# kowallus/mbgc

Hardware: AMD Instinct MI355X
Metric: input Gbases/s (compress hot path, -m1: match-finding + stream emission) (higher is better)
Workload: dtype u8

## Files before the change

### mbgc_amd/binding.py

```python
import ctypes as C
import os

import numpy as np

HERE = os.path.dirname(os.path.abspath(__file__))
LIB_PATH = os.environ.get("MBGC_HIP_LIB", os.path.join(HERE, "libmbgc_hip.so"))
NO_LOCK = 2 ** 64 - 1
SKIPPED = 2 ** 64 - 1
STREAM_NAMES = ("literals", "mapOff", "mapOff5th", "mapLen", "gapDelta", "flags")
KERNEL_FAMILIES = ("load", "insert", "probe", "emit2", "resolve", "stitch", "emit")

EXPORTS = """swsem_last_error swsem_device_count swsem_device_numa_node swsem_create swsem_destroy swsem_set_stream swsem_synchronize
swsem_disable_sliding_window swsem_set_sliding_window_size swsem_disable_circular_buffer swsem_get_ref_length
swsem_get_loading_position swsem_get_loaded_ref_length swsem_get_max_ref_length swsem_get_sliding_window_size swsem_get_dropped_bytes swsem_set_position
swsem_acquire_lock swsem_release_lock swsem_get_K swsem_get_hash_size swsem_load_ref swsem_load_ref_dev
swsem_load_separator swsem_finalize_targets swsem_revcomp_dev swsem_match swsem_match_batch_dev swsem_batch_counts swsem_batch_matches
swsem_batch_fingerprint swsem_emit_params_default swsem_emit swsem_emit_batch swsem_emit_batch_begin swsem_emit_batch_begin_spec swsem_emit_batch_end swsem_emit_select swsem_emit_result swsem_emit_set_host_copy swsem_emit_unmatched swsem_emit_pack_dev swsem_emit_pack_dev_on swsem_emit_counters swsem_debug_copy_ref swsem_debug_write_ref swsem_debug_copy_ht swsem_debug_emit_stats
swsem_profile_enable swsem_profile_get swsem_batch_stats swsem_dev_malloc swsem_dev_free swsem_dev_upload swsem_dev_download swsem_dev_copy swsem_decode_contigs_dev swsem_emit_verify
swsem_create_decoder swsem_decode_plan_chain_dev swsem_decode_fill_range_dev swsem_decode_load_dev""".split()


class SpecFinalize(C.Structure):
    _fields_ = [("ntargets", C.c_int), ("ext_dev", C.c_void_p), ("ext_len", C.POINTER(C.c_uint64)), ("addSep", C.c_int), ("sep", C.c_int),
                ("lazySeparator", C.c_int), ("lockPos", C.POINTER(C.c_uint64)), ("loadedAfter", C.POINTER(C.c_uint64)),
# ... 122 lines not shown
        L.swsem_profile_get.argtypes = [vp, C.POINTER(C.c_double), pu64]
        L.swsem_batch_stats.argtypes = [vp, pu64]
        _lib = L
    return _lib


def _chk(rc):
    if rc != 0:
        raise SwsemError("swsem error %d: %s" % (rc, lib().swsem_last_error().decode()))


def _bytes_ptr(a):
    a = np.ascontiguousarray(a, dtype=np.uint8)
    return a, a.ctypes.data_as(C.c_void_p)


def emit_params(mode=1, **over):
    p = EmitParams()
    lib().swsem_emit_params_default(C.byref(p), mode)
    for k, v in over.items():
        setattr(p, k, v)
    return p


class SlidingWindowSparseEMMatcher:

    def __init__(self, max_ref_len, L=32, k1=16, k2=1, skip_margin=16, device=0):
        self.h = C.c_void_p()
        _chk(lib().swsem_create(C.byref(self.h), max_ref_len, L, k1, k2, skip_margin, device))

    def close(self):
        if getattr(self, "h", None):
            lib().swsem_destroy(self.h)
            self.h = None

    def __del__(self):
        self.close()

    def disable_sliding_window(self): lib().swsem_disable_sliding_window(self.h)
    def set_sliding_window_size(self, f): lib().swsem_set_sliding_window_size(self.h, f)
    def disable_circular_buffer(self): lib().swsem_disable_circular_buffer(self.h)
    def ref_length(self): return lib().swsem_get_ref_length(self.h)
    def loading_position(self): return lib().swsem_get_loading_position(self.h)
    def loaded_ref_length(self): return lib().swsem_get_loaded_ref_length(self.h)
    def max_ref_length(self): return lib().swsem_get_max_ref_length(self.h)
    def sliding_window_size(self): return lib().swsem_get_sliding_window_size(self.h)
    def dropped_bytes(self): return lib().swsem_get_dropped_bytes(self.h)

    def emit_stats(self):
        out = (C.c_uint64 * 8)()
        lib().swsem_debug_emit_stats.argtypes = [C.c_void_p, C.POINTER(C.c_uint64)]
        _chk(lib().swsem_debug_emit_stats(self.h, out))
        return {"foreign_boundary_steps": int(out[4]), "blocks_not_accepted": int(out[5]), "groups_replayed": int(out[6]),
                "blocks_given_up": int(out[7])}
    def set_position(self, pos, laps): lib().swsem_set_position(self.h, pos, laps)
    def acquire_lock(self): return lib().swsem_acquire_lock(self.h)
    def release_lock(self, v): _chk(lib().swsem_release_lock(self.h, v)); return 0
    def hash_size(self): return lib().swsem_get_hash_size(self.h)
    def K(self): return lib().swsem_get_K(self.h)
    def set_stream(self, stream_ptr): _chk(lib().swsem_set_stream(self.h, stream_ptr))
    def synchronize(self): _chk(lib().swsem_synchronize(self.h))

    def load_ref(self, text, load_rc=False, add_sep=True, sep=0):
        a, p = _bytes_ptr(text)
        _chk(lib().swsem_load_ref(self.h, p, a.size, int(load_rc), int(add_sep), sep))

    def load_ref_dev(self, dev_ptr, n, load_rc=False, add_sep=True, sep=0):
        _chk(lib().swsem_load_ref_dev(self.h, dev_ptr, n, int(load_rc), int(add_sep), sep))

    def load_separator(self, sep=0): _chk(lib().swsem_load_separator(self.h, sep))

    def finalize_targets(self, ext_ptrs, ext_lens, locks, lazy=True, add_sep=True, sep=0):
        n = len(ext_lens)
        ptrs = (C.c_void_p * n)(*[int(p) for p in ext_ptrs])
        lens = np.ascontiguousarray(ext_lens, dtype=np.uint64)
        lk = np.ascontiguousarray(locks, dtype=np.uint64)
        out = np.zeros(n, dtype=np.uint64)
        P = C.POINTER(C.c_uint64)
        _chk(lib().swsem_finalize_targets(self.h, n, ptrs, lens.ctypes.data_as(P), int(add_sep), sep, int(lazy),
                                          lk.ctypes.data_as(P), out.ctypes.data_as(P)))
        return out
    def revcomp_dev(self, src_ptr, n, dst_ptr): _chk(lib().swsem_revcomp_dev(self.h, src_ptr, n, dst_ptr))

    def match(self, q, min_len=32, lock=NO_LOCK):
        a, p = _bytes_ptr(q)
        out, n = C.c_void_p(), C.c_uint64()
        _chk(lib().swsem_match(self.h, p, a.size, min_len, lock, C.byref(out), C.byref(n)))
        if n.value == 0:
            return np.zeros((0, 3), dtype=np.uint64)
        return np.ctypeslib.as_array(C.cast(out, C.POINTER(C.c_uint64)), shape=(n.value, 3)).copy()

    def match_batch_dev(self, dev_ptr, offsets, min_len=32, locks=None):
        offs = np.ascontiguousarray(offsets, dtype=np.uint64)
        n = offs.size - 1
        lk = None
        if locks is not None:
            lk = np.ascontiguousarray(locks, dtype=np.uint64)
            assert lk.size == n
        _chk(lib().swsem_match_batch_dev(self.h, dev_ptr, offs.ctypes.data_as(C.POINTER(C.c_uint64)), n, min_len,
                                         lk.ctypes.data_as(C.POINTER(C.c_uint64)) if lk is not None else None))
        self._batch_n = n

    def batch_counts(self):
        out = np.zeros(self._batch_n, dtype=np.uint64)
        _chk(lib().swsem_batch_counts(self.h, out.ctypes.data_as(C.POINTER(C.c_uint64))))
        return out

# ... 190 lines not shown
```

### mbgc_amd/csrc/swsem_emit.hip

```cpp
#include "swsem_device.h"
#include "../../include/mbgc_swsem.h"

namespace swk {

constexpr int EMIT_THREADS = 1024;
constexpr uint8_t MATCH_MARK = 0xA5;
constexpr int MAX_EXTEND_MATCH_LEFT_LENGTH = 1 << 24;

struct EMatch {
    uint64_t posSrc, len, posDest, lp;
};

struct EmitContig {
    uint64_t qoff, n;
    uint64_t matchBase;
    uint64_t lock;
    uint64_t scratchBase;
    uint64_t streamBase[SWSEM_NSTREAMS];
    uint32_t cap;
    uint32_t chunk0;
    int32_t factor;
    uint32_t span0;
    int64_t processed, targetIdx;
};

struct EmitOut {
    uint64_t size[SWSEM_NSTREAMS];
    uint64_t unmatchedChars;
    uint64_t extMatched, extMismatches, totalMatched, removed, nmatches;
};

struct LongCopy { uint8_t *dst; const uint8_t *src; uint64_t len; };
constexpr uint32_t LONG_COPY_CAP = 4096;
constexpr uint32_t LONG_COPY_MIN = 32768;

struct EmitView {
    const uint8_t *ref, *qbuf;
    const Match *matches;
    const uint32_t *matchCount;
    uint64_t pos1, refLength, maxRefLength;
    const uint64_t *loaded; uint32_t nLoaded;
    swsem_emit_params_t p;
    EMatch *em;
    uint64_t *next0;
    uint8_t *removed;
    uint32_t *keepIdx;
    uint32_t *meta;
    uint32_t *corr;
    unsigned long long *pairMask;
    unsigned long long *litBits;
    unsigned long long *metaBad;
    uint32_t *sz;
    uint32_t *ofs;
    uint32_t *chunkCnt;
    const uint32_t *chunkOwner;
    const uint32_t *spanOwner;
    uint32_t ncontigs;
    uint64_t *packBase;
    uint8_t *arena;
    struct LongCopy *longCopies;
    uint32_t *longCount;
    EmitOut *out;
};

constexpr uint32_t META_SKIPOFF = 1, META_HASGAP = 2, META_ISGAP = 4, META_GSTART = 8, META_GMID = 16, META_GEND = 32;

__device__ __forceinline__ bool paired(uint64_t aSrc, uint64_t aDst, uint64_t bSrc, uint64_t bDst) {
    return aSrc + bDst == bSrc + aDst;
}

__device__ __forceinline__ int sym5(uint8_t c) {
    return c == 'A' ? 0 : c == 'C' ? 1 : c == 'G' ? 2 : c == 'T' ? 3 : c == 'N' ? 4 : -1;
}
__device__ __forceinline__ uint8_t mismatch2code(uint8_t actual, uint8_t mismatch) {
    const int a = sym5(actual), b = sym5(mismatch);
    if (actual == mismatch || a < 0 || b < 0) return mismatch;
    const uint32_t rows[5] = {0 | 2u << 3 | 0u << 6 | 1u << 9 | 3u << 12, 1 | 0u << 3 | 2u << 6 | 0u << 9 | 3u << 12,
                              0 | 2u << 3 | 0u << 6 | 1u << 9 | 3u << 12, 1 | 0u << 3 | 2u << 6 | 0u << 9 | 3u << 12,
                              1 | 2u << 3 | 3u << 6 | 0u << 9 | 0u << 12};
    return (uint8_t) ((rows[a] >> (3 * b)) & 7u);
}

__device__ __forceinline__ uint64_t loaded_pos(const EmitView &v, uint64_t pos) {
    const uint64_t span = v.refLength - 1;
    const uint64_t back = v.loaded[v.nLoaded - 1];
    while (pos + span < back) pos += span;
    return pos;
}

template <int NT>
__device__ uint32_t block_scan(uint32_t x, uint32_t *lds, uint32_t *total) {
    const uint32_t lane = threadIdx.x & (WAVE - 1), w = threadIdx.x / WAVE;
    uint32_t inc = x;
    for (int d = 1; d < WAVE; d <<= 1) {
        const uint32_t y = (uint32_t) __shfl_up((int) inc, d);
        if ((int) lane >= d) inc += y;
    }
    __syncthreads();
    if (lane == WAVE - 1) lds[w] = inc;
    __syncthreads();
    if (threadIdx.x == 0) {
        uint32_t run = 0;
        for (int i = 0; i < NT / WAVE; i++) { const uint32_t t = lds[i]; lds[i] = run; run += t; }
// ... 285 lines not shown
                                    (gs ? META_GSTART : 0) | (gm ? META_GMID : 0) | (ge ? META_GEND : 0) | (gapByte << 8);
                metaV = wl32(mw, k, metaV);
                corrV = wl32(isGap ? (uint32_t) st.gapStartIdx : (uint32_t) j, k, corrV);
            }
        }
        if (WRITE && lane < cnt) {
            v.meta[cg.scratchBase + jl] = metaV;
            v.corr[cg.scratchBase + jl] = corrV;
        }
        st.nxA = st.nxB;
        st.nxB = 0;
    }
}


__device__ __forceinline__ bool mrec_equal(const MetaRec &a, const MetaRec &b) {
    uint32_t ra, rb;
    __builtin_memcpy(&ra, a.rel, 4); __builtin_memcpy(&rb, b.rel, 4);
    uint64_t d = (a.claimed ^ b.claimed) | (uint64_t) (a.gapStartIdx ^ b.gapStartIdx) | (uint64_t) (a.gapEndIdx ^ b.gapEndIdx) |
                 (uint64_t) (a.flags ^ b.flags) | (uint64_t) (ra ^ rb);
#pragma unroll
    for (int e = 0; e < MNX; e++) d |= a.val[e] ^ b.val[e];
    return d == 0;
}

__device__ __forceinline__ void mrec_store(MetaRec *dst, unsigned long long claimed, bool cur, int gs, int ge, const int (&nxPos)[MNX],
                                           const uint64_t (&nxVal)[MNX], bool overflow, int J) {
    uint32_t r[MNX]; uint64_t x[MNX];
#pragma unroll
    for (int e = 0; e < MNX; e++) { r[e] = nxPos[e] >= J ? (uint32_t) (nxPos[e] - J) : 0xFFu; x[e] = nxPos[e] >= J ? nxVal[e] : 0; }
    auto cx = [&](int a, int b) {
        if (r[a] > r[b]) { const uint32_t t = r[a]; r[a] = r[b]; r[b] = t; const uint64_t u = x[a]; x[a] = x[b]; x[b] = u; }
    };
    cx(0, 1); cx(2, 3); cx(0, 2); cx(1, 3); cx(1, 2);
    MetaRec R;
    R.claimed = claimed; R.gapStartIdx = gs; R.gapEndIdx = ge;
    R.flags = (cur ? MREC_CUR : 0u) | (overflow ? MREC_OVERFLOW : 0u);
#pragma unroll
    for (int e = 0; e < MNX; e++) { R.rel[e] = (uint8_t) r[e]; R.val[e] = x[e]; }
    *dst = R;
}

struct MetaSpan { uint32_t gk; int n, B0; bool live; };
__device__ __forceinline__ MetaSpan meta_span(const EmitView &v, const EmitContig *__restrict__ cgs) {
    MetaSpan sp;
    sp.gk = v.spanOwner[blockIdx.x];
    const EmitOut o = v.out[sp.gk];
    sp.n = (int) o.nmatches;
    sp.B0 = (int) (blockIdx.x - cgs[sp.gk].span0) * MSPAN;
    sp.live = o.unmatchedChars != UINT64_MAX && sp.B0 < sp.n;
    return sp;
}

__global__ void __launch_bounds__(CH) k_emit_meta_regions(EmitView v, const EmitContig *__restrict__ cgs) {
    if (!v.p.lazyDecompressionSupport) return;
    const uint32_t gk = v.chunkOwner[blockIdx.x];
    const EmitContig cg = cgs[gk];
    const uint32_t gx = blockIdx.x - cg.chunk0;
    const EmitOut o = v.out[gk];
    if (o.unmatchedChars == UINT64_MAX) return;
    const uint64_t t = (uint64_t) gx * CH + threadIdx.x;
    if (t >= o.nmatches) return;
    const uint64_t lp = loaded_pos(v, v.em[cg.scratchBase + t].posSrc);
    v.em[cg.scratchBase + t].lp = lp;
    uint32_t lo = 0, hi = v.nLoaded;
    while (lo < hi) { const uint32_t mid = (lo + hi) / 2; if (v.loaded[mid] <= lp) lo = mid + 1; else hi = mid; }
    v.next0[cg.scratchBase + t] = lo == v.nLoaded ? UINT64_MAX : v.loaded[lo];
}

__global__ void __launch_bounds__(MLANES) k_emit_meta_masks(EmitView v, const EmitContig *__restrict__ cgs) {
    __shared__ uint64_t skey[MPAD_SIZE], slp[MPAD_SIZE];
    const MetaSpan sp = meta_span(v, cgs);
    if (!sp.live) return;
    const EmitContig cg = cgs[sp.gk];
    const int n = sp.n, B0 = sp.B0, tid = (int) threadIdx.x;
    const int P1 = B0 + MSPAN < n ? B0 + MSPAN : n;
    const int PK = P1 + WAVE < n ? P1 + WAVE : n;
    const EMatch *E = v.em + cg.scratchBase;
    const bool lazy = v.p.lazyDecompressionSupport != 0;
    const int depth = v.p.gapDepthOffsetEncoding;
    for (int i = tid; i < ((PK - B0 + WAVE - 1) & ~(WAVE - 1)); i += MLANES) {
        const int m = B0 + i;
        bool lit0 = false;
        if (m < PK) {
            const EMatch e = E[m];
            const uint64_t side = e.posSrc > cg.lock ? 1u : (e.posSrc < cg.lock ? 2u : 0u);
            skey[mpad(i)] = ((e.posSrc - e.posDest) << 2) | side;
            slp[mpad(i)] = e.lp;
            const uint64_t nxt = m + 1 < n ? E[m + 1].posDest : cg.n;
            lit0 = nxt - (uint32_t) (e.posDest + e.len) == 0;
        }
        const unsigned long long lb = __ballot(lit0);
        if ((tid & (WAVE - 1)) == 0 && m < P1) v.litBits[(size_t) cg.chunk0 * (CH / WAVE) + (size_t) (m / WAVE)] = lb;
    }
    __syncthreads();
    for (int i = tid; i < P1 - B0; i += MLANES) {
        const int m = B0 + i;
        const int gCnt = n - m - 1 < depth ? n - m - 1 : depth;
        const uint64_t kj = skey[mpad(i)];
        const uint64_t own = lazy ? v.next0[cg.scratchBase + m] : UINT64_MAX;
        unsigned long long pm = 0;
#pragma unroll 8
        for (int g = 1; g <= WAVE; g++) {
            const int x = mpad(g <= gCnt ? i + g : i);
            const bool ok = (g <= gCnt) & (skey[x] == kj) & ((slp[x] < own) | !lazy);
            pm |= (unsigned long long) ok << (g - 1);
        }
        v.pairMask[cg.scratchBase + m] = pm;
    }
}

__global__ void __launch_bounds__(MLANES) k_emit_meta_spec(EmitView v, const EmitContig *__restrict__ cgs, MetaRec *__restrict__ recs, int warm,
                                                          unsigned long long *__restrict__ stats) {
    __shared__ uint64_t spm[MPAD_SIZE], sown[MPAD_SIZE];
    __shared__ unsigned long long slit[MPAD_N / WAVE + 2];
    const MetaSpan sp = meta_span(v, cgs);
    if (!sp.live) return;
    const EmitContig cg = cgs[sp.gk];
    const int n = sp.n, B0 = sp.B0, tid = (int) threadIdx.x;
    const int P0 = B0 >= MWARM ? B0 - MWARM : 0;
    const int P1 = B0 + MSPAN < n ? B0 + MSPAN : n;
    const EMatch *E = v.em + cg.scratchBase;
    const bool lazy = v.p.lazyDecompressionSupport != 0, ext = v.p.enableExtensionsWithMismatches != 0;
    const int depth = v.p.gapDepthOffsetEncoding, depthMism = v.p.gapDepthMismatchesEncoding;
    const int PK = P1 + WAVE < n ? P1 + WAVE : n;
    for (int i = tid; i < PK - P0; i += MLANES) {
        if (P0 + i < P1) spm[mpad(i)] = v.pairMask[cg.scratchBase + P0 + i];
        sown[mpad(i)] = lazy ? v.next0[cg.scratchBase + P0 + i] : 0;
    }
    if (tid < MPAD_N / WAVE + 2) {
        const int w = P0 / WAVE + tid;
        slit[tid] = w * WAVE < P1 ? v.litBits[(size_t) cg.chunk0 * (CH / WAVE) + (size_t) w] : 0;
    }
    __syncthreads();
    const int j0 = B0 + tid * MB;
    const bool active = j0 < n;
    const int j1 = j0 + MB < n ? j0 + MB : n;
    unsigned long long claimed = 0;
    bool cur = false, overflow = false;
    int gs = -1, ge = -1;
    int nxPos[MNX]; uint64_t nxVal[MNX];
#pragma unroll
    for (int e = 0; e < MNX; e++) { nxPos[e] = -1; nxVal[e] = 0; }
    MetaRec *myRecs = recs + ((size_t) cg.chunk0 * (CH / MB) + (size_t) (j0 / MB)) * 2;
    for (int s = 0; s < MWARM + MB; s++) {
        const int j = j0 - MWARM + s;
        if (s == MWARM && active) mrec_store(myRecs, claimed, cur, gs, ge, nxPos, nxVal, overflow, j0);
        if (!active || j < j0 - warm || j < 0 || j >= j1) continue;
        const int i = j - P0;
        if (ext && j == ge) { gs = -1; ge = -1; }
        const bool skipOffset = cur;
        const int gCnt = n - j - 1 < depth ? n - j - 1 : depth;
        const bool rule = !lazy && gs == -1 && ((slit[i / WAVE] >> (i & (WAVE - 1))) & 1);
        const unsigned long long taken = claimed | (rule ? 1ull : 0ull);
        unsigned long long em = spm[mpad(i)] & ~taken;
        uint64_t inherited = 0;
#pragma unroll
        for (int e = 0; e < MNX; e++) if (nxPos[e] == j) { inherited = nxVal[e]; nxPos[e] = -1; }
        uint64_t nextj = 0;
        if (lazy) {
            nextj = sown[mpad(i)];
            if (inherited && inherited != nextj) {
                nextj = inherited;
                atomicAdd(&stats[4], 1ull);
                const EMatch mj = E[j];
                em = 0;
                for (int g = 1; g <= gCnt; g++) {
                    const EMatch c = E[j + g];
                    const bool pw = paired(mj.posSrc, mj.posDest, c.posSrc, c.posDest) &&
                                    ((mj.posSrc > cg.lock && c.posSrc > cg.lock) || (mj.posSrc < cg.lock && c.posSrc < cg.lock));
                    if (pw && c.lp < nextj) em |= 1ull << (g - 1);
                }
                em &= ~taken;
            }
        }
        uint32_t gapByte = 0;
        if (em) {
            const int gf = __builtin_ctzll(em) + 1;
            const unsigned long long below = gf > 1 ? ((1ull << (gf - 1)) - 1) : 0ull;
            gapByte = (uint32_t) (gf - __popcll(taken & below));
            claimed |= 1ull << (gf - 1);
            if (lazy && nextj != sown[mpad(i + gf)]) {
                bool put = false;
#pragma unroll
                for (int e = 0; e < MNX; e++) if (!put && nxPos[e] < 0) { nxPos[e] = j + gf; nxVal[e] = nextj; put = true; }
                overflow |= !put;
            }
            if (ext && ge <= j + gf && gf <= depthMism) { gs = j; ge = j + gf; }
        }
        cur = claimed & 1ull;
        claimed >>= 1;
        if (j >= j0) {
            const bool s0 = gs == j, e0 = ge == j + 1, m0 = gs < j && j + 1 < ge;
            const bool isGap = s0 || m0 || e0;
            const uint32_t mw = (skipOffset ? META_SKIPOFF : 0) | (gCnt ? META_HASGAP : 0) | (isGap ? META_ISGAP : 0) |
                                (s0 ? META_GSTART : 0) | (m0 ? META_GMID : 0) | (e0 ? META_GEND : 0) | (gapByte << 8);
            v.meta[cg.scratchBase + j] = mw;
            v.corr[cg.scratchBase + j] = (uint32_t) (isGap ? gs : j);
        }
    }
    if (active) mrec_store(myRecs + 1, claimed, cur, gs, ge, nxPos, nxVal, overflow, j1);
    if (active && overflow) atomicAdd(&stats[7], 1ull);
}

__global__ void __launch_bounds__(WAVE) k_emit_meta_check(EmitView v, const EmitContig *__restrict__ cgs, const MetaRec *__restrict__ recs,
                                                          unsigned long long *__restrict__ stats) {
    constexpr int CPW = WAVE * MB / CH;
    const uint32_t gk = v.chunkOwner[blockIdx.x];
    const EmitContig cg = cgs[gk];
    const uint32_t gx = blockIdx.x - cg.chunk0;
    if (gx % CPW) return;
    const EmitOut o = v.out[gk];
    if (o.unmatchedChars == UINT64_MAX) return;
    const int64_t n = (int64_t) o.nmatches, nblk = (n + MB - 1) / MB;
    const int64_t b = (int64_t) (gx / CPW) * WAVE + threadIdx.x;
    if (b - (int64_t) threadIdx.x >= nblk) return;
    const MetaRec *R0 = recs + (size_t) cg.chunk0 * (CH / MB) * 2;
    bool bad = false;
    if (b < nblk) {
        const MetaRec S = R0[2 * b], F = R0[2 * b + 1];
        bad = ((S.flags | F.flags) & MREC_OVERFLOW) != 0;
        if (b > 0 && !bad) bad = !mrec_equal(S, R0[2 * b - 1]);
    }
    const unsigned long long mb = __ballot(bad);
    if (threadIdx.x == 0) {
        v.metaBad[cg.chunk0 + gx / CPW] = mb;
        if (mb) atomicAdd(&stats[5], (unsigned long long) __popcll(mb));
    }
}

__device__ __forceinline__ void mrec_expand(const MetaRec &R, MetaRun &st) {
    st.claimed = rfl64(R.claimed); st.curClaimed = (rfl32(R.flags) & MREC_CUR) != 0;
    st.gapStartIdx = (int64_t) rfl64((uint64_t) R.gapStartIdx); st.gapEndIdx = (int64_t) rfl64((uint64_t) R.gapEndIdx);
    st.nxA = 0; st.nxB = 0;
#pragma unroll
// ... 743 lines not shown
```

### mbgc_amd/csrc/swsem_runtime.hip

```cpp
#include "../../include/mbgc_swsem.h"
#include "swsem_kernels.hip"
#include "swsem_resolve4.hip"
#include "swsem_emit.hip"
#include "swsem_decode.hip"

#include <algorithm>
#include <cctype>
#include <chrono>
#include <mutex>
#include <cstdarg>
#include <cstdio>
#include <cstdlib>
#include <cstring>
#include <deque>
#include <string>
#include <vector>

using namespace swk;

#include "swsem_runtime_state.h"
#include "swsem_runtime_streams.h"
#include "swsem_runtime_loader.h"
#include "swsem_runtime_match.h"
#include "swsem_runtime_emit.h"
// ... 290 lines not shown
    HIPCHK(hipGetLastError());
    return SWSEM_OK;
}

int swsem_debug_copy_ref(swsem_t *h, uint64_t from, uint64_t n, uint8_t *out) {
    HIPCHK(hipStreamSynchronize(h->stream));
    HIPCHK(hipMemcpy(out, h->ref + from, n, hipMemcpyDeviceToHost));
    return SWSEM_OK;
}

int swsem_debug_write_ref(swsem_t *h, uint64_t from, uint64_t n, const uint8_t *in) { MATCHER_ONLY(h);
    if (from + n > h->maxRefLength) return fail(SWSEM_EINVAL, "swsem_debug_write_ref: beyond the buffer");
    HIPCHK(hipStreamSynchronize(h->stream));
    HIPCHK(hipStreamSynchronize(h->stream2));
    HIPCHK(hipMemcpy(h->ref + from, in, n, hipMemcpyHostToDevice));
    {
        const uint64_t s0 = from >= (uint64_t) h->K ? (from - h->K + 1) >> h->k1ord : 0, s1 = (from + n + ((1ull << h->k1ord) - 1)) >> h->k1ord;
        if (h->tags && s1 > s0) HIPCHK(hipMemset(h->tags + s0, 0, (s1 - s0) * sizeof(uint16_t)));
    }
    return SWSEM_OK;
}

int swsem_debug_copy_ht(swsem_t *h, uint32_t *out) { MATCHER_ONLY(h);
    DevBuf<uint32_t> tmp;
    int r = tmp.reserve(h->hash_size);
    if (r) return r;
    k_ht_low_words<<<dim3((h->hash_size + 255) / 256), dim3(256), 0, h->stream>>>(h->ht, tmp.p, h->hash_size, h->fpBits);
    HIPCHK(hipStreamSynchronize(h->stream));
    HIPCHK(hipMemcpy(out, tmp.p, (size_t) h->hash_size * 4, hipMemcpyDeviceToHost));
    return SWSEM_OK;
}

int swsem_debug_block_times(swsem_t *h, uint64_t *out, uint64_t cap, uint64_t *n) { MATCHER_ONLY(h);
    uint64_t nb = 0;
    for (auto &c : h->contigs) nb += c.nrb;
    *n = nb;
    if (nb > cap) nb = cap;
    std::vector<BlockRec> tmp(nb);
    HIPCHK(hipStreamSynchronize(h->stream));
    if (nb) HIPCHK(hipMemcpy(tmp.data(), h->dRecs.p, nb * sizeof(BlockRec), hipMemcpyDeviceToHost));
    for (uint64_t i = 0; i < nb; i++) { out[3 * i] = tmp[i].cycles; out[3 * i + 1] = tmp[i].visits; out[3 * i + 2] = tmp[i].emits; }
    return SWSEM_OK;
}

int swsem_debug_emit_stats(swsem_t *h, uint64_t out[8]) { MATCHER_ONLY(h);
    HIPCHK(hipDeviceSynchronize());
    for (int k = 0; k < 8; k++) out[k] = 0;
    for (auto &E : h->slot) {
        if (!E.dEStat.p || !E.statZeroed) continue;
        unsigned long long t[8];
        HIPCHK(hipMemcpy(t, E.dEStat.p, sizeof t, hipMemcpyDeviceToHost));
        for (int k = 0; k < 8; k++) out[k] += t[k];
    }
    return SWSEM_OK;
}

#ifdef SWSEM_DIAG_PHASES
int swsem_debug_phases(swsem_t *h, uint64_t *out) {
    HIPCHK(hipStreamSynchronize(h->stream));
    unsigned long long z[8] = {0};
    HIPCHK(hipMemcpyFromSymbol(out, HIP_SYMBOL(swk::g_diag), sizeof z));
    HIPCHK(hipMemcpyToSymbol(HIP_SYMBOL(swk::g_diag), z, sizeof z));
    return SWSEM_OK;
}
#endif

int swsem_profile_enable(swsem_t *h, int on) {
    h->drain_events();
    h->prof = on != 0;
    memset(h->profMs, 0, sizeof h->profMs);
    memset(h->profN, 0, sizeof h->profN);
    return SWSEM_OK;
}

int swsem_profile_get(swsem_t *h, double ms[SWSEM_K_COUNT], uint64_t n[SWSEM_K_COUNT]) {
    h->drain_events();
    for (int i = 0; i < SWSEM_K_COUNT; i++) { ms[i] = h->profMs[i]; n[i] = h->profN[i]; }
    return SWSEM_OK;
}

int swsem_batch_stats(swsem_t *h, uint64_t s[9]) { MATCHER_ONLY(h);
    if (!h->batchValid) return fail(SWSEM_EINVAL, "no batch results");
    for (int i = 0; i < 9; i++) s[i] = h->stats[i];
    return SWSEM_OK;
}

void swsem_emit_params_default(swsem_emit_params_t *p, int mode) {
    memset(p, 0, sizeof(*p));
    p->enableExtensionsWithMismatches = 1;
    p->mismatchesWithExclusion = 1;
    p->lazyDecompressionSupport = 1;
    p->enable40bitReference = 0;
    p->frugal64bitLenEncoding = 1;
    p->gapDepthOffsetEncoding = 64;
    p->gapDepthMismatchesEncoding = 2;
    p->gapBreakingMatchMinLength = 256;
    p->mmsMatchBonus = 50;
    p->mmsMismatchPenalty = 50;
    p->mmsMismatchesScoreThreshold = 500;
    p->mmsMismatchesInitialScore = 125;
    p->allowedTargetsOutrunForDissimilarContigs = 1;
    p->minimalLengthForDissimilarContigs = 1024;
    p->unmatchedFractionFactorTweakForDissimilarContigs = 16;
    if (mode == 0) {
        p->allowedTargetsOutrunForDissimilarContigs = 4;
        p->unmatchedFractionFactorTweakForDissimilarContigs = 32;
// ... 231 lines not shown
```

### mbgc_amd/csrc/swsem_runtime_emit.h

```cpp
namespace {

int end_slot(swsem *h, int si) {
    EmitSlot &E = h->slot[si];
    if (!E.outstanding) return SWSEM_OK;
    HIPCHK(hipSetDevice(h->device));
    { int d = run_phase2b(h, E, false); if (d) return d; }
    HIPCHK(hipEventSynchronize(E.evDone));
    E.outstanding = false;
    const int n = E.emitN;
    E.eout.assign((const EmitOut *) E.pinE.p, (const EmitOut *) E.pinE.p + n);
    uint64_t tot = 0;
    E.hostStreamOff.assign((size_t) n * SWSEM_NSTREAMS, 0);
    for (int k = 0; k < n; k++)
        for (int st = 0; st < SWSEM_NSTREAMS; st++) {
            if (E.eout[k].unmatchedChars == UINT64_MAX) E.eout[k].size[st] = 0;
            E.hostStreamOff[(size_t) k * SWSEM_NSTREAMS + st] = tot;
            tot += E.eout[k].size[st];
        }
    E.packedBytes = tot;
    E.hostStreamsValid = false;
    if (h->emitHostCopy) {
        int r = E.next_host_streams(tot + 1);
        if (r) return r;
        if (tot) HIPCHK(hipMemcpyAsync(E.hostStreams().p, E.dEArena.p, tot, hipMemcpyDeviceToHost, h->s3()));
        HIPCHK(hipStreamSynchronize(h->s3()));
        E.hostStreamsValid = true;
    }
    return SWSEM_OK;
}


int emit_layout(swsem *h, EmitSlot &E, int n, const int *contigIdx, const uint64_t *lockPos, const int *factor,
                const int64_t *processed, const int64_t *targetIdx, uint64_t &rows, uint64_t &arena) {
    E.ecg.assign(n, EmitContig());
    std::vector<int> &which = E.ewhich;
    which.assign(n, 0);
    rows = 0; arena = 0;
    E.chunkOwner.clear(); E.spanOwner.clear();
    for (int k = 0; k < n; k++) {
        const int c = contigIdx ? contigIdx[k] : k;
        if (c < 0 || c >= (int) h->contigs.size()) return fail(SWSEM_EINVAL, "swsem_emit: no contig %d in the batch", c);
        which[k] = c;
        EmitContig &e = E.ecg[k];
        const Contig &cg = h->contigs[c];
        const uint64_t nm = cg.n / (h->minLen ? h->minLen : 1) + 2;
        e.qoff = cg.qoff; e.n = cg.n; e.matchBase = cg.matchBase;
        e.lock = lockPos ? lockPos[k] : UINT64_MAX;
        e.scratchBase = rows;
        e.cap = (uint32_t) (nm + 2);
        rows += e.cap;
        e.chunk0 = (uint32_t) E.chunkOwner.size();
        E.chunkOwner.insert(E.chunkOwner.end(), (e.cap + CH - 1) / CH, (uint32_t) k);
        e.span0 = (uint32_t) E.spanOwner.size();
        E.spanOwner.insert(E.spanOwner.end(), (e.cap + MSPAN - 1) / MSPAN, (uint32_t) k);
        e.factor = factor ? factor[k] : 128;
        e.processed = processed ? processed[k] : 0;
        e.targetIdx = targetIdx ? targetIdx[k] : 0;
        const uint64_t szs[SWSEM_NSTREAMS] = {cg.n + nm + 16, 4 * nm + 16, nm + 16, 14 * nm + 16, nm + 16, cg.n + 2 * nm + 16};
        for (int st = 0; st < SWSEM_NSTREAMS; st++) { e.streamBase[st] = arena; arena += (szs[st] + 15) & ~15ull; }
    }
    return SWSEM_OK;
}

int emit_reserve(swsem *h, EmitSlot &E, int n, uint64_t rows, uint64_t arena, uint64_t nLoaded) {
    h->capN = std::max<uint64_t>(h->capN, (uint64_t) n); h->capRows = std::max(h->capRows, rows); h->capArena = std::max(h->capArena, arena);
    if (nLoaded + 1 > h->capLoaded) h->capLoaded = std::max<uint64_t>(4096, 2 * (nLoaded + 1));
    h->capChunks = std::max<uint64_t>(h->capChunks, E.chunkOwner.size());
    const uint64_t N = h->capN, R = h->capRows, A = h->capArena, Cn = h->capChunks;
    int r;
    if ((r = E.dECg.reserve(N)) || (r = E.dEOut.reserve(N)) || (r = E.dEWhich.reserve(N)) || (r = E.dEM.reserve(R)) ||
        (r = E.dENext0.reserve(R)) || (r = E.dERm.reserve(R)) ||
        (r = E.dEKeep.reserve(R)) || (r = E.dEMeta.reserve(R)) || (r = E.dECorr.reserve(R)) ||
        (r = E.dESz.reserve(R * 6)) || (r = E.dEOfs.reserve(R * 6)) || (r = E.dEArena.reserve(A)) || (r = E.dELoaded.reserve(h->capLoaded)) ||
        (r = E.dEStat.reserve(8)) || (r = E.dELong.reserve(LONG_COPY_CAP)) || (r = E.dELongCount.reserve(4)) || (r = E.dEPm.reserve(R)) ||
        (r = E.dELit.reserve((size_t) Cn * (CH / WAVE))) || (r = E.dEBad.reserve(Cn)) || (r = E.dEOwner.reserve(Cn)) || (r = E.dESpanOwner.reserve(Cn)) ||
        (r = E.dEStates.reserve((size_t) Cn * (CH / MB) * 2)) || (r = E.dEChunk.reserve((size_t) Cn * 6)) ||
        (r = E.dEPack.reserve((size_t) N * SWSEM_NSTREAMS)))
        return r;
    if (!E.statZeroed) { HIPCHK(hipMemsetAsync(E.dEStat.p, 0, 8 * sizeof(unsigned long long), h->stream)); E.statZeroed = true; }
    return SWSEM_OK;
}

int emit_upload_tables(swsem *h, EmitSlot &E, int n, const uint64_t *refExtLoadedPos, uint64_t nLoaded, const swsem_spec_finalize_t *spec) {
    hipStream_t up = h->streamUp;
    int r;
    if (!h->roundTopFresh) HIPCHK(hipEventRecord(h->evRoundTop, h->stream));
    h->roundTopFresh = false;
    HIPCHK(hipStreamWaitEvent(up, h->evRoundTop, 0));
    if ((r = upload(h, E.dEOwner.p, E.chunkOwner.data(), E.chunkOwner.size() * sizeof(uint32_t), up))) return r;
    if ((r = upload(h, E.dESpanOwner.p, E.spanOwner.data(), E.spanOwner.size() * sizeof(uint32_t), up))) return r;
    if ((r = upload(h, E.dECg.p, E.ecg.data(), n * sizeof(EmitContig), up)) || (r = upload(h, E.dEWhich.p, E.ewhich.data(), n * sizeof(int), up))) return r;
    E.eloaded.assign(refExtLoadedPos, refExtLoadedPos + nLoaded);
    if ((r = upload(h, E.dELoaded.p, E.eloaded.data(), nLoaded * sizeof(uint64_t), up))) return r;
    if (spec) {
        if ((r = h->dGate.reserve(4)) || (r = h->dPred.reserve(2 * (size_t) n + 64))) return r;
        if ((r = upload(h, h->dPred.p, spec->predExt, n, up)) || (r = upload(h, h->dPred.p + n, spec->predRC, n, up))) return r;
    }
    return flush_copies(h);
}

EmitView emit_book(swsem *h, EmitSlot &E, int si, const swsem_emit_params_t *p, int n, uint64_t nLoaded) {
    EmitView v;
    v.ref = h->ref; v.qbuf = h->qdev; v.matches = h->dMatches.p; v.matchCount = h->dMatchCount.p;
    v.pos1 = (uint64_t) h->ld.pos1; v.refLength = h->refLength(); v.maxRefLength = h->maxRefLength;
    v.loaded = E.dELoaded.p; v.nLoaded = (uint32_t) nLoaded; v.p = *p;
    v.em = E.dEM.p; v.next0 = E.dENext0.p; v.removed = E.dERm.p; v.keepIdx = E.dEKeep.p;
    v.meta = E.dEMeta.p; v.corr = E.dECorr.p; v.sz = E.dESz.p; v.arena = E.dEArena.p; v.out = E.dEOut.p;
    v.packBase = E.dEPack.p;
    v.pairMask = E.dEPm.p; v.litBits = E.dELit.p; v.metaBad = E.dEBad.p;
    v.longCopies = E.dELong.p; v.longCount = E.dELongCount.p;
    v.ofs = E.dEOfs.p;
    v.chunkCnt = E.dEChunk.p;
    v.chunkOwner = E.dEOwner.p; v.spanOwner = E.dESpanOwner.p;
    v.ncontigs = (uint32_t) n;
    E.v2b = v; E.grid2b = (uint32_t) E.chunkOwner.size(); E.n2b = n;
    E.donePending = true;
    h->latest = si; h->selected = -1;
    E.outstanding = true; E.refGuarded = false; E.emitN = n; E.emitPos1 = (uint64_t) h->ld.pos1; E.qdev = h->qdev; E.params = *p;
    E.emitLaps = h->ld.laps;
    uint64_t lm = UINT64_MAX; bool all = true;
    for (int k = 0; k < n; k++) { if (E.ecg[k].lock == UINT64_MAX) all = false; else lm = std::min(lm, E.ecg[k].lock); }
    E.lockMin = all ? lm : UINT64_MAX;
    E.packedBytes = 0; E.hostStreamsValid = false;
    E.deferred2b = false;
    return v;
}

int spec_plan(swsem *h, const swsem_spec_finalize_t *spec, const uint32_t *gate, bool &planned) {
    h->specMode = true;
    int r = finalize_impl(h, spec->ntargets, spec->ext_dev, spec->ext_len, spec->addSep, spec->sep, spec->lazySeparator, spec->lockPos,
                          spec->loadedAfter, gate, true);
    h->specMode = false;
    planned = r == SWSEM_OK;
    if (r == SWSEM_ESPEC) return SWSEM_OK;
    if (r) return r;
    return prepare_inserts(h, h->streamUp);
}

int emit_pass1(swsem *h, EmitSlot &E, const EmitView &v, int n) {
    const dim3 grid2(E.grid2b);
    int r;
    HIPCHK(hipEventRecord(h->evTables, h->streamUp));
    HIPCHK(hipStreamWaitEvent(h->stream, h->evTables, 0));
    hipStream_t sP = h->stream;
    h->mark(SWSEM_K_EMIT, true, sP);
    k_emit_p1_removed<<<grid2, dim3(CH), 0, sP>>>(v, E.dECg.p, E.dEWhich.p);
    k_emit_p1_scan<<<dim3(n), dim3(CH), 0, sP>>>(v, E.dECg.p, E.dEWhich.p);
    k_emit_p1_compact<<<grid2, dim3(CH), 0, sP>>>(v, E.dECg.p, E.dEWhich.p);
    k_emit_p1_finish<<<dim3(n), dim3(CH), 0, sP>>>(v, E.dECg.p);
    h->mark(SWSEM_K_EMIT, false, sP);
    HIPCHK(hipGetLastError());
    if ((r = queue_counts(h, n * sizeof(EmitOut), sP))) return r;
    if ((r = download(h, h->pin.p + h->pinExtraAt, E.dEOut.p, n * sizeof(EmitOut), sP)) || (r = flush_copies(h))) return r;
    HIPCHK(hipEventRecord(h->evP1, sP));
    return SWSEM_OK;
}

int emit_pairing(swsem *h, EmitSlot &E, const EmitView &v, int n) {
    const dim3 grid2(E.grid2b), spans((uint32_t) E.spanOwner.size());
    const size_t outBytes = n * sizeof(EmitOut);
    int r = E.pinE.reserve(outBytes, std::max<size_t>(2 * outBytes, 1 << 20));
    if (r) return r;
    HIPCHK(hipStreamWaitEvent(h->streamAux, h->evP1, 0));
    h->mark(SWSEM_K_EMIT2, true, h->streamAux);
    k_emit_meta_regions<<<grid2, dim3(CH), 0, h->streamAux>>>(v, E.dECg.p);
    k_emit_meta_masks<<<spans, dim3(MLANES), 0, h->streamAux>>>(v, E.dECg.p);
    k_emit_meta_spec<<<spans, dim3(MLANES), 0, h->streamAux>>>(v, E.dECg.p, E.dEStates.p, h->sw.metaWarm, E.dEStat.p);
    HIPCHK(hipEventRecord(h->evMeta, h->streamAux));
    h->metaPending = true;
    k_emit_meta_check<<<grid2, dim3(WAVE), 0, h->streamAux>>>(v, E.dECg.p, E.dEStates.p, E.dEStat.p);
    k_emit_meta_stitch<<<dim3(n), dim3(WAVE), 0, h->streamAux>>>(v, E.dECg.p, E.dEStates.p, E.dEStat.p);
    h->mark(SWSEM_K_EMIT2, false, h->streamAux);
    HIPCHK(hipEventRecord(E.evMetaDone, h->streamAux));
    HIPCHK(hipGetLastError());
    return SWSEM_OK;
}

int spec_gate(swsem *h, EmitSlot &E, const swsem_spec_finalize_t *spec, uint32_t *gate, int n, bool planned, bool &queued, bool &exchanged) {
    k_spec_verify<<<1, 256, 0, h->stream>>>(E.dEOut.p, E.dECg.p, n, h->dPred.p, h->dPred.p + n, spec->factor, spec->rcFactor, gate);
    if (spec->veto || !planned) HIPCHK(hipMemsetAsync(gate, 0, sizeof(uint32_t), h->stream));
    if (spec->exchange) {
        if (spec->exchange(spec->exchange_ctx, 0, gate, (void *) h->stream)) return fail(SWSEM_EHIP, "speculative finalize: the exchange between the replicas failed");
        exchanged = true;
    }
    if (planned) {
        int r = launch_inserts(h, gate);
        if (r) return r;
        queued = true;
    }
    return SWSEM_OK;
}

bool spec_verdict(swsem *h, const EmitSlot &E, const swsem_spec_finalize_t *spec, int n, bool exchanged) {
    bool ok = !spec->veto;
    for (int k = 0; k < n && ok; k++) {
        const uint64_t un = E.eout[k].unmatchedChars, len = E.ecg[k].n;
        ok = un != UINT64_MAX && (un * (uint64_t) spec->factor > len) == (spec->predExt[k] != 0) &&
             (un * (uint64_t) spec->rcFactor > len) == (spec->predRC[k] != 0);
    }
    if (exchanged) ok = spec->exchange(spec->exchange_ctx, 1, nullptr, (void *) h->stream) == 1 && ok;
    return ok;
}

int emit_begin_impl(swsem *h, const swsem_emit_params_t *p, int n, const int *contigIdx, const uint64_t *lockPos,
                    const int *factor, const int64_t *processed, const int64_t *targetIdx,
                    const uint64_t *refExtLoadedPos, uint64_t nLoaded, const swsem_spec_finalize_t *spec, int *applied) {
    HIPCHK(hipSetDevice(h->device));
    if (applied) *applied = 0;
    if (spec && spec->ntargets <= 0) spec = nullptr;
    const int si = h->latest ^ 1;
    { int e = end_slot(h, si); if (e) return e; }
    EmitSlot &E = h->slot[si];
    if (!h->batchValid) return fail(SWSEM_EINVAL, "swsem_emit: no match results on the handle");
    if (n <= 0) return fail(SWSEM_EINVAL, "swsem_emit: empty request");
    if (p->lazyDecompressionSupport && nLoaded == 0) return fail(SWSEM_EINVAL, "swsem_emit: lazy mode needs refExtLoadedPosArr");
    if (p->gapDepthOffsetEncoding > 64 || p->gapDepthOffsetEncoding < 0)
        return fail(SWSEM_EINVAL, "gapDepthOffsetEncoding %d out of range (MAX_GAP_DEPTH / 2)", p->gapDepthOffsetEncoding);
    int r;
    uint64_t rows, arena;
    if ((r = emit_layout(h, E, n, contigIdx, lockPos, factor, processed, targetIdx, rows, arena)) ||
// ... 30 lines not shown
```

### mbgc_amd/csrc/swsem_runtime_state.h

```cpp
#define SWSEM_ESPEC (-100)

namespace {

thread_local std::string g_err;
int fail(int code, const char *fmt, ...) {
    char buf[512];
    va_list ap;
    va_start(ap, fmt);
    vsnprintf(buf, sizeof buf, fmt, ap);
    va_end(ap);
    g_err = buf;
    return code;
}
#define HIPCHK(x) do { hipError_t e_ = (x); if (e_ != hipSuccess) return fail(SWSEM_EHIP, "%s: %s", #x, hipGetErrorString(e_)); } while (0)

constexpr uint64_t REF_SHIFT = 1;
constexpr int SW_WIDTH_FACTOR = 16;
constexpr uint64_t REF_SLACK = 256;
constexpr uint64_t COPY_WGS = 2048;
constexpr uint32_t EMIT_THIN_MAX = 512;
constexpr uint32_t RB_MIN = 2048 / RBU;
constexpr uint32_t CAND_MAX = 4096;
constexpr uint64_t CAND_BYTES = 128ull << 20;
constexpr int NSTATS = 16;
// ... 69 lines not shown
        ePrev = eCur; eCur = epoch;
        pos1 = REF_SHIFT;
        samplingPos = REF_SHIFT;
    }
};

struct Switches {
    bool seqResolve = false;
    bool simt = true;
    uint32_t rbFixed = 0;
    int overlapFixed = -1;
    uint32_t profMask = ~0u;
    int metaWarm = swk::MWARM;
    bool lapTags = true;
    bool streamCalib = true;
    bool streamDebug = false;
    bool debugStats = false;
};
Switches read_switches() {
    Switches s;
    if (const char *e = getenv("SWSEM_RESOLVE")) s.seqResolve = strcmp(e, "seq") == 0;
    if (const char *e = getenv("SWSEM_CHAINS")) s.simt = atoi(e) != 1;
    if (const char *e = getenv("SWSEM_RB")) { int x = atoi(e); if (x >= 1 && x <= 256) s.rbFixed = (uint32_t) x * (1024 / RBU); }
    if (const char *e = getenv("SWSEM_OVERLAP")) { int x = atoi(e); if (x >= 0 && x <= swk::OVERLAP_MAX) s.overlapFixed = x; }
    if (const char *e = getenv("SWSEM_PROF_FAMS")) s.profMask = (uint32_t) strtoul(e, nullptr, 0);
    if (const char *e = getenv("SWSEM_META_WARM")) s.metaWarm = std::min(swk::MWARM, std::max(0, atoi(e)));
    if (const char *e = getenv("SWSEM_LAP_TAGS")) s.lapTags = atoi(e) != 0;
    if (const char *e = getenv("SWSEM_STREAM_CALIB")) s.streamCalib = atoi(e) != 0;
    s.streamDebug = getenv("SWSEM_STREAM_DEBUG") != nullptr;
    s.debugStats = getenv("SWSEM_DEBUG_STATS") != nullptr;
    return s;
}

struct PreparedInserts {
    size_t np = 0, nc = 0, nb = 0, ne = 0;
    bool beside = false;
    uint64_t nSamples = 0, nEdge = 0, copyBlocks = 0;
    const InsertPiece *dPieces = nullptr, *dEdge = nullptr;
    const uint64_t *dFirst = nullptr, *dCFirst = nullptr, *dEFirst = nullptr;
    const CopyPiece *dCopies = nullptr;
    const BytePiece *dBytes = nullptr;
};

struct EmitSlot {
    DevBuf<EmitContig> dECg;
    DevBuf<EmitOut> dEOut;
    DevBuf<int> dEWhich;
    DevBuf<uint32_t> dEOwner, dESpanOwner;
    DevBuf<EMatch> dEM;
    DevBuf<uint64_t> dENext0, dELoaded, dEPack;
    DevBuf<uint8_t> dERm, dEArena;
    DevBuf<uint32_t> dEKeep, dEMeta, dECorr, dESz, dEOfs, dEChunk;
    DevBuf<MetaRec> dEStates;
    DevBuf<unsigned long long> dEStat, dEPm, dELit, dEBad;
    DevBuf<LongCopy> dELong;
    DevBuf<uint32_t> dELongCount;
    bool statZeroed = false;
    std::vector<EmitContig> ecg;
    std::vector<uint32_t> chunkOwner, spanOwner;
    std::vector<int> ewhich;
    std::vector<uint64_t> eloaded;
    std::vector<EmitOut> eout;
    Event evDone;
    Event evMetaDone;
    bool outstanding = false, refGuarded = false;
    bool donePending = false;
    bool deferred2b = false, waitFin2b = false;
    EmitView v2b; uint32_t grid2b = 0; int n2b = 0;
    const uint8_t *qdev = nullptr;
    swsem_emit_params_t params;
    uint64_t emitPos1 = 0;
    uint64_t lockMin = UINT64_MAX;
    int emitLaps = 0;
    int emitN = 0;
    PinBuf pinE;
    PinBuf hostHalf[2];
    int hostAt = 0;
    PinBuf &hostStreams() { return hostHalf[hostAt]; }
    int next_host_streams(size_t n) { hostAt ^= 1; return hostStreams().reserve(n, n + n / 2 + 4096, hipHostMallocDefault); }
    std::vector<uint64_t> hostStreamOff;
    bool hostStreamsValid = false;
    uint64_t packedBytes = 0;
};

}

struct swsem {
    int device = 0;
    hipStream_t stream = nullptr;
    bool ownStream = false;
    Switches sw;
    uint8_t *ref = nullptr;
    ht_entry *ht = nullptr;
    uint8_t *lut = nullptr;
    uint16_t *tags = nullptr;
    bool useTags = true;
    LoaderState ld;
    uint64_t maxRefLength = 0;
    int L = 0, K = 0, k1 = 0, skipMargin = 0, k1ord = 0;
    uint32_t hash_size = 0, mask = 0;
    uint64_t swSize = 0;
    bool circular = true;
    int fpBits = 0;
    uint64_t hostProbes = 0;
    bool deferInserts = false;
    bool specMode = false;
    DevBuf<uint32_t> dGate;
// ... 137 lines not shown
```

Before: 56.33.

## Fuse meta regions, masks and spec kernels into one chained pairing kernel

Replaces three kernels (region lookup, pair-mask build, speculative chain) with one kernel per span. Loaded-position lookup, binary search for next region, pair masks and literal bits are computed in registers and shared memory instead of round-tripping through the global pairMask/litBits buffers. The cost is recomputing the warm-up prefix per span, a lock-step binary search across rounds, and extra loaded_pos calls on the rare inherited-boundary path. It also removes two device buffers and adds a profiling script and debug stats fields.

```diff
diff --git a/mbgc_amd/binding.py b/mbgc_amd/binding.py
--- a/mbgc_amd/binding.py
+++ b/mbgc_amd/binding.py
@@ -198,7 +198,7 @@
         lib().swsem_debug_emit_stats.argtypes = [C.c_void_p, C.POINTER(C.c_uint64)]
         _chk(lib().swsem_debug_emit_stats(self.h, out))
         return {"foreign_boundary_steps": int(out[4]), "blocks_not_accepted": int(out[5]), "groups_replayed": int(out[6]),
-                "blocks_given_up": int(out[7])}
+                "blocks_given_up": int(out[7]), "span_matches": int(out[0]), "warm_up_matches": int(out[1])}
     def set_position(self, pos, laps): lib().swsem_set_position(self.h, pos, laps)
     def acquire_lock(self): return lib().swsem_acquire_lock(self.h)
     def release_lock(self, v): _chk(lib().swsem_release_lock(self.h, v)); return 0
diff --git a/mbgc_amd/csrc/swsem_emit.hip b/mbgc_amd/csrc/swsem_emit.hip
--- a/mbgc_amd/csrc/swsem_emit.hip
+++ b/mbgc_amd/csrc/swsem_emit.hip
@@ -47,8 +47,6 @@
     uint32_t *keepIdx;
     uint32_t *meta;
     uint32_t *corr;
-    unsigned long long *pairMask;
-    unsigned long long *litBits;
     unsigned long long *metaBad;
     uint32_t *sz;
     uint32_t *ofs;
@@ -440,85 +438,83 @@
     return sp;
 }
 
-__global__ void __launch_bounds__(CH) k_emit_meta_regions(EmitView v, const EmitContig *__restrict__ cgs) {
-    if (!v.p.lazyDecompressionSupport) return;
-    const uint32_t gk = v.chunkOwner[blockIdx.x];
-    const EmitContig cg = cgs[gk];
-    const uint32_t gx = blockIdx.x - cg.chunk0;
-    const EmitOut o = v.out[gk];
-    if (o.unmatchedChars == UINT64_MAX) return;
-    const uint64_t t = (uint64_t) gx * CH + threadIdx.x;
-    if (t >= o.nmatches) return;
-    const uint64_t lp = loaded_pos(v, v.em[cg.scratchBase + t].posSrc);
-    v.em[cg.scratchBase + t].lp = lp;
-    uint32_t lo = 0, hi = v.nLoaded;
-    while (lo < hi) { const uint32_t mid = (lo + hi) / 2; if (v.loaded[mid] <= lp) lo = mid + 1; else hi = mid; }
-    v.next0[cg.scratchBase + t] = lo == v.nLoaded ? UINT64_MAX : v.loaded[lo];
-}
-
-__global__ void __launch_bounds__(MLANES) k_emit_meta_masks(EmitView v, const EmitContig *__restrict__ cgs) {
+constexpr int MROUNDS = (MPAD_N + MLANES - 1) / MLANES;
+__global__ void __launch_bounds__(MLANES) k_emit_meta_chain(EmitView v, const EmitContig *__restrict__ cgs, MetaRec *__restrict__ recs, int warm,
+                                                           unsigned long long *__restrict__ stats) {
     __shared__ uint64_t skey[MPAD_SIZE], slp[MPAD_SIZE];
-    const MetaSpan sp = meta_span(v, cgs);
-    if (!sp.live) return;
-    const EmitContig cg = cgs[sp.gk];
-    const int n = sp.n, B0 = sp.B0, tid = (int) threadIdx.x;
-    const int P1 = B0 + MSPAN < n ? B0 + MSPAN : n;
-    const int PK = P1 + WAVE < n ? P1 + WAVE : n;
-    const EMatch *E = v.em + cg.scratchBase;
-    const bool lazy = v.p.lazyDecompressionSupport != 0;
-    const int depth = v.p.gapDepthOffsetEncoding;
-    for (int i = tid; i < ((PK - B0 + WAVE - 1) & ~(WAVE - 1)); i += MLANES) {
-        const int m = B0 + i;
-        bool lit0 = false;
-        if (m < PK) {
-            const EMatch e = E[m];
-            const uint64_t side = e.posSrc > cg.lock ? 1u : (e.posSrc < cg.lock ? 2u : 0u);
-            skey[mpad(i)] = ((e.posSrc - e.posDest) << 2) | side;
-            slp[mpad(i)] = e.lp;
-            const uint64_t nxt = m + 1 < n ? E[m + 1].posDest : cg.n;
-            lit0 = nxt - (uint32_t) (e.posDest + e.len) == 0;
-        }
-        const unsigned long long lb = __ballot(lit0);
-        if ((tid & (WAVE - 1)) == 0 && m < P1) v.litBits[(size_t) cg.chunk0 * (CH / WAVE) + (size_t) (m / WAVE)] = lb;
-    }
-    __syncthreads();
-    for (int i = tid; i < P1 - B0; i += MLANES) {
-        const int m = B0 + i;
-        const int gCnt = n - m - 1 < depth ? n - m - 1 : depth;
-        const uint64_t kj = skey[mpad(i)];
-        const uint64_t own = lazy ? v.next0[cg.scratchBase + m] : UINT64_MAX;
-        unsigned long long pm = 0;
-#pragma unroll 8
-        for (int g = 1; g <= WAVE; g++) {
-            const int x = mpad(g <= gCnt ? i + g : i);
-            const bool ok = (g <= gCnt) & (skey[x] == kj) & ((slp[x] < own) | !lazy);
-            pm |= (unsigned long long) ok << (g - 1);
-        }
-        v.pairMask[cg.scratchBase + m] = pm;
-    }
-}
-
-__global__ void __launch_bounds__(MLANES) k_emit_meta_spec(EmitView v, const EmitContig *__restrict__ cgs, MetaRec *__restrict__ recs, int warm,
-                                                          unsigned long long *__restrict__ stats) {
-    __shared__ uint64_t spm[MPAD_SIZE], sown[MPAD_SIZE];
-    __shared__ unsigned long long slit[MPAD_N / WAVE + 2];
+    __shared__ unsigned long long slit[MROUNDS * MLANES / WAVE];
     const MetaSpan sp = meta_span(v, cgs);
     if (!sp.live) return;
     const EmitContig cg = cgs[sp.gk];
     const int n = sp.n, B0 = sp.B0, tid = (int) threadIdx.x;
     const int P0 = B0 >= MWARM ? B0 - MWARM : 0;
     const int P1 = B0 + MSPAN < n ? B0 + MSPAN : n;
+    const int PK = P1 + WAVE < n ? P1 + WAVE : n;
+    const int cnt = PK - P0;
     const EMatch *E = v.em + cg.scratchBase;
     const bool lazy = v.p.lazyDecompressionSupport != 0, ext = v.p.enableExtensionsWithMismatches != 0;
     const int depth = v.p.gapDepthOffsetEncoding, depthMism = v.p.gapDepthMismatchesEncoding;
-    const int PK = P1 + WAVE < n ? P1 + WAVE : n;
-    for (int i = tid; i < PK - P0; i += MLANES) {
-        if (P0 + i < P1) spm[mpad(i)] = v.pairMask[cg.scratchBase + P0 + i];
-        sown[mpad(i)] = lazy ? v.next0[cg.scratchBase + P0 + i] : 0;
-    }
-    if (tid < MPAD_N / WAVE + 2) {
-        const int w = P0 / WAVE + tid;
-        slit[tid] = w * WAVE < P1 ? v.litBits[(size_t) cg.chunk0 * (CH / WAVE) + (size_t) w] : 0;
+    uint64_t lpk[MROUNDS], own[MROUNDS];
+    uint32_t lo[MROUNDS], hi[MROUNDS];
+#pragma unroll
+    for (int k = 0; k < MROUNDS; k++) {
+        lpk[k] = 0; lo[k] = 0; hi[k] = 0;
+        if (k * MLANES >= cnt) continue;
+        const int i = tid + k * MLANES, m = P0 + i;
+        bool lit0 = false;
+        if (m < PK) {
+            const EMatch e = E[m];
+            const uint64_t side = e.posSrc > cg.lock ? 1u : (e.posSrc < cg.lock ? 2u : 0u);
+            skey[mpad(i)] = ((e.posSrc - e.posDest) << 2) | side;
+            if (lazy) { lpk[k] = loaded_pos(v, e.posSrc); hi[k] = v.nLoaded; }
+            slp[mpad(i)] = lpk[k];
+            const uint64_t nxt = m + 1 < n ? E[m + 1].posDest : cg.n;
+            lit0 = nxt - (uint32_t) (e.posDest + e.len) == 0;
+        }
+        const unsigned long long lb = __ballot(lit0);
+        if ((tid & (WAVE - 1)) == 0) slit[i / WAVE] = lb;
+    }
+    const int levels = lazy ? 32 - __builtin_clz(v.nLoaded) : 0;
+    for (int l = 0; l < levels; l++) {
+#pragma unroll
+        for (int k = 0; k < MROUNDS; k++) {
+            const bool open = lo[k] < hi[k];
+            const uint32_t mid = open ? (lo[k] + hi[k]) / 2 : 0;
+            const bool right = v.loaded[mid] <= lpk[k];
+            lo[k] = open && right ? mid + 1 : lo[k];
+            hi[k] = open && !right ? mid : hi[k];
+        }
+    }
+#pragma unroll
+    for (int k = 0; k < MROUNDS; k++) {
+        const int m = P0 + tid + k * MLANES;
+        own[k] = 0;
+        if (!lazy || m >= PK) continue;
+        own[k] = lo[k] == v.nLoaded ? UINT64_MAX : v.loaded[lo[k]];
+        if (m >= B0 && m < P1) {
+            v.em[cg.scratchBase + m].lp = lpk[k];
+            v.next0[cg.scratchBase + m] = own[k];
+        }
+    }
+    __syncthreads();
+#pragma unroll
+    for (int k = 0; k < MROUNDS; k++) {
+        if (k * MLANES >= cnt) continue;
+        const int i = tid + k * MLANES, m = P0 + i;
+        unsigned long long pm = 0;
+        if (m < P1) {
+            const int gCnt = n - m - 1 < depth ? n - m - 1 : depth;
+            const uint64_t kj = skey[mpad(i)];
+            const uint64_t bound = lazy ? own[k] : UINT64_MAX;
+#pragma unroll 8
+            for (int g = 1; g <= WAVE; g++) {
+                const int x = mpad(g <= gCnt ? i + g : i);
+                const bool ok = (g <= gCnt) & (skey[x] == kj) & ((slp[x] < bound) | !lazy);
+                pm |= (unsigned long long) ok << (g - 1);
+            }
+        }
+        __syncthreads();
+        if (m < PK) { skey[mpad(i)] = pm; slp[mpad(i)] = own[k]; }
     }
     __syncthreads();
     const int j0 = B0 + tid * MB;
@@ -541,13 +537,13 @@
         const int gCnt = n - j - 1 < depth ? n - j - 1 : depth;
         const bool rule = !lazy && gs == -1 && ((slit[i / WAVE] >> (i & (WAVE - 1))) & 1);
         const unsigned long long taken = claimed | (rule ? 1ull : 0ull);
-        unsigned long long em = spm[mpad(i)] & ~taken;
+        unsigned long long em = skey[mpad(i)] & ~taken;
         uint64_t inherited = 0;
 #pragma unroll
         for (int e = 0; e < MNX; e++) if (nxPos[e] == j) { inherited = nxVal[e]; nxPos[e] = -1; }
         uint64_t nextj = 0;
         if (lazy) {
-            nextj = sown[mpad(i)];
+            nextj = slp[mpad(i)];
             if (inherited && inherited != nextj) {
                 nextj = inherited;
                 atomicAdd(&stats[4], 1ull);
@@ -557,7 +553,7 @@
                     const EMatch c = E[j + g];
                     const bool pw = paired(mj.posSrc, mj.posDest, c.posSrc, c.posDest) &&
                                     ((mj.posSrc > cg.lock && c.posSrc > cg.lock) || (mj.posSrc < cg.lock && c.posSrc < cg.lock));
-                    if (pw && c.lp < nextj) em |= 1ull << (g - 1);
+                    if (pw && loaded_pos(v, c.posSrc) < nextj) em |= 1ull << (g - 1);
                 }
                 em &= ~taken;
             }
@@ -568,7 +564,7 @@
             const unsigned long long below = gf > 1 ? ((1ull << (gf - 1)) - 1) : 0ull;
             gapByte = (uint32_t) (gf - __popcll(taken & below));
             claimed |= 1ull << (gf - 1);
-            if (lazy && nextj != sown[mpad(i + gf)]) {
+            if (lazy && nextj != slp[mpad(i + gf)]) {
                 bool put = false;
 #pragma unroll
                 for (int e = 0; e < MNX; e++) if (!put && nxPos[e] < 0) { nxPos[e] = j + gf; nxVal[e] = nextj; put = true; }
diff --git a/mbgc_amd/csrc/swsem_runtime.hip b/mbgc_amd/csrc/swsem_runtime.hip
--- a/mbgc_amd/csrc/swsem_runtime.hip
+++ b/mbgc_amd/csrc/swsem_runtime.hip
@@ -366,6 +366,7 @@
         HIPCHK(hipMemcpy(t, E.dEStat.p, sizeof t, hipMemcpyDeviceToHost));
         for (int k = 0; k < 8; k++) out[k] += t[k];
     }
+    out[0] = swk::MSPAN; out[1] = swk::MWARM;
     return SWSEM_OK;
 }
 
diff --git a/mbgc_amd/csrc/swsem_runtime_emit.h b/mbgc_amd/csrc/swsem_runtime_emit.h
--- a/mbgc_amd/csrc/swsem_runtime_emit.h
+++ b/mbgc_amd/csrc/swsem_runtime_emit.h
@@ -72,8 +72,8 @@
         (r = E.dENext0.reserve(R)) || (r = E.dERm.reserve(R)) ||
         (r = E.dEKeep.reserve(R)) || (r = E.dEMeta.reserve(R)) || (r = E.dECorr.reserve(R)) ||
         (r = E.dESz.reserve(R * 6)) || (r = E.dEOfs.reserve(R * 6)) || (r = E.dEArena.reserve(A)) || (r = E.dELoaded.reserve(h->capLoaded)) ||
-        (r = E.dEStat.reserve(8)) || (r = E.dELong.reserve(LONG_COPY_CAP)) || (r = E.dELongCount.reserve(4)) || (r = E.dEPm.reserve(R)) ||
-        (r = E.dELit.reserve((size_t) Cn * (CH / WAVE))) || (r = E.dEBad.reserve(Cn)) || (r = E.dEOwner.reserve(Cn)) || (r = E.dESpanOwner.reserve(Cn)) ||
+        (r = E.dEStat.reserve(8)) || (r = E.dELong.reserve(LONG_COPY_CAP)) || (r = E.dELongCount.reserve(4)) ||
+        (r = E.dEBad.reserve(Cn)) || (r = E.dEOwner.reserve(Cn)) || (r = E.dESpanOwner.reserve(Cn)) ||
         (r = E.dEStates.reserve((size_t) Cn * (CH / MB) * 2)) || (r = E.dEChunk.reserve((size_t) Cn * 6)) ||
         (r = E.dEPack.reserve((size_t) N * SWSEM_NSTREAMS)))
         return r;
@@ -107,7 +107,7 @@
     v.em = E.dEM.p; v.next0 = E.dENext0.p; v.removed = E.dERm.p; v.keepIdx = E.dEKeep.p;
     v.meta = E.dEMeta.p; v.corr = E.dECorr.p; v.sz = E.dESz.p; v.arena = E.dEArena.p; v.out = E.dEOut.p;
     v.packBase = E.dEPack.p;
-    v.pairMask = E.dEPm.p; v.litBits = E.dELit.p; v.metaBad = E.dEBad.p;
+    v.metaBad = E.dEBad.p;
     v.longCopies = E.dELong.p; v.longCount = E.dELongCount.p;
     v.ofs = E.dEOfs.p;
     v.chunkCnt = E.dEChunk.p;
@@ -163,9 +163,7 @@
     if (r) return r;
     HIPCHK(hipStreamWaitEvent(h->streamAux, h->evP1, 0));
     h->mark(SWSEM_K_EMIT2, true, h->streamAux);
-    k_emit_meta_regions<<<grid2, dim3(CH), 0, h->streamAux>>>(v, E.dECg.p);
-    k_emit_meta_masks<<<spans, dim3(MLANES), 0, h->streamAux>>>(v, E.dECg.p);
-    k_emit_meta_spec<<<spans, dim3(MLANES), 0, h->streamAux>>>(v, E.dECg.p, E.dEStates.p, h->sw.metaWarm, E.dEStat.p);
+    k_emit_meta_chain<<<spans, dim3(MLANES), 0, h->streamAux>>>(v, E.dECg.p, E.dEStates.p, h->sw.metaWarm, E.dEStat.p);
     HIPCHK(hipEventRecord(h->evMeta, h->streamAux));
     h->metaPending = true;
     k_emit_meta_check<<<grid2, dim3(WAVE), 0, h->streamAux>>>(v, E.dECg.p, E.dEStates.p, E.dEStat.p);
diff --git a/mbgc_amd/csrc/swsem_runtime_state.h b/mbgc_amd/csrc/swsem_runtime_state.h
--- a/mbgc_amd/csrc/swsem_runtime_state.h
+++ b/mbgc_amd/csrc/swsem_runtime_state.h
@@ -145,7 +145,7 @@
     DevBuf<uint8_t> dERm, dEArena;
     DevBuf<uint32_t> dEKeep, dEMeta, dECorr, dESz, dEOfs, dEChunk;
     DevBuf<MetaRec> dEStates;
-    DevBuf<unsigned long long> dEStat, dEPm, dELit, dEBad;
+    DevBuf<unsigned long long> dEStat, dEBad;
     DevBuf<LongCopy> dELong;
     DevBuf<uint32_t> dELongCount;
     bool statZeroed = false;
diff --git a/profiles/pairing_gate.py b/profiles/pairing_gate.py
--- /dev/null
+++ b/profiles/pairing_gate.py
@@ -0,0 +1,27 @@
+#!/usr/bin/env python3
+import csv
+import glob
+import sys
+
+f = glob.glob(sys.argv[1] + "/**/*kernel_trace.csv", recursive=True)[0]
+rows = sorted(csv.DictReader(open(f)), key=lambda r: int(r["Start_Timestamp"]))
+idx = [i for i, r in enumerate(rows) if "k_resolve_blocks" in r["Kernel_Name"]]
+PAIR = ("k_emit_meta_spec", "k_emit_meta_chain")
+print("step  insert_end  main_last_end  pairing_first_start  pairing_end  next_resolve  resolve-pairing  resolve-main  pairing_kernels_us")
+for a, b in zip(idx[-12:-1], idx[-11:]):
+    t0 = int(rows[a]["Start_Timestamp"])
+    qmain = rows[a].get("Queue_Id")
+    seg = rows[a + 1:b]
+    ins = [int(r["End_Timestamp"]) for r in seg if "k_insert_multi" in r["Kernel_Name"]]
+    main = [int(r["End_Timestamp"]) for r in seg if r.get("Queue_Id") == qmain]
+    pend = [int(r["End_Timestamp"]) for r in seg if any(p in r["Kernel_Name"] for p in PAIR)]
+    pst = [int(r["Start_Timestamp"]) for r in seg if any(p in r["Kernel_Name"] for p in ("k_emit_meta_regions", "k_emit_meta_chain"))]
+    durs = ["%s %.1f" % (r["Kernel_Name"].split("(")[0].split("::")[-1], (int(r["End_Timestamp"]) - int(r["Start_Timestamp"])) / 1e3)
+            for r in seg if "k_emit_meta_" in r["Kernel_Name"]]
+    nxt = int(rows[b]["Start_Timestamp"])
+    u = lambda x: (x - t0) / 1e3
+    if not (ins and main and pend and pst):
+        print("step without insertion / pairing kernels", len(seg))
+        continue
+    print("%4d  %9.1f  %12.1f  %12.1f  %10.1f  %11.1f  %8.1f  %8.1f   %s" % (a, u(max(ins)), u(max(main)), u(min(pst)), u(max(pend)), u(nxt),
+                                                                 (nxt - max(pend)) / 1e3, (nxt - max(main)) / 1e3, " | ".join(durs)))
```

New measurement: 55.66. 1.2% lower.
